# konstantineder/montecarlo-risk-engine

Hardware: AMD Instinct MI355X
Metric: path-steps/sec at 1M paths x 250 steps; PV/CVA rel-error vs CPU ref (higher is better)
Workload: dtype f64

## Files before the change

### montecarlo-risk-engine_amd/csrc/kf_common.h

```cpp
#pragma once
#include <cstddef>
#include "mcx_device.h"



enum { FA_EXP = 1, FA_AFFINE = 2 };
struct FAtom {
    int32_t reg, parts;
    double a, d, b, c0, c1;
};
struct FTerm { double w; FAtom atom; };
enum { FE_SAME_NUM = 2 };
struct FEvent {
    int32_t kind, flags;
    int32_t term_begin, term_end;
    int32_t coeff_off, row;
    int32_t ns, sidx;
    int32_t init_state, n_states;
    double strike, sign;
    double aux[4];
    FAtom num, x;
};
struct FMetricOp {
    int32_t ns, m;
// ... 385 lines not shown
        if (row >= 0) {
#pragma unroll
            for (int q = 0; q < PPL; ++q) if (live[q]) a.expo[(int64_t)row * a.ld_out + i[q]] = e[q];
        }
    }
    if (flags & FD_METRIC) {
        const double thr = FD(thr);
        double u[PPL];
#pragma unroll
        for (int q = 0; q < PPL; ++q) u[q] = dev_thr(e[q], thr);
        if (flags & FD_PROFILE) {
            const int rp = FD(rec_profile);
            double up[PPL], un[PPL];
#pragma unroll
            for (int q = 0; q < PPL; ++q) { up[q] = fmax(u[q], 0.0); un[q] = fmin(u[q], 0.0); }
            lean_record<PPL>(up, live, rp, a.n_rec, first_tile, lds);
            lean_record<PPL>(un, live, rp + 1, a.n_rec, first_tile, lds);
        }
        if (flags & FD_CVA) {
            const double sb = FD(s_b), sc0 = FD(s_c0), sc1 = FD(s_c1);
            const int sr = FD(s_reg);
            double sp[PPL], cs[PPL];
#pragma unroll
            for (int q = 0; q < PPL; ++q) sp[q] = sb * mcx_exp_tab(fma(sc1, reg[q][sr], sc0), etab, ec);
            cond_surv(cs);
#pragma unroll
            for (int q = 0; q < PPL; ++q) cva[q] = fma(fmax(u[q], 0.0), sp[q] * (1.0 - cs[q]), cva[q]);
        }
    }
}

#undef FD

int mcx_launch_kf_lean(const FusedArgs& a, const mcx_sim_desc& sd, int n_cu, bool inject, bool simulate, hipStream_t s);
```

### montecarlo-risk-engine_amd/csrc/kf_fused.hip

```cpp
#include "kf_common.h"

#include <algorithm>
#include <type_traits>
#include <cmath>
#include <cstdlib>

namespace {

template <int NSLOT, int SIG, int NNS, int NSTA, bool STORE>
__device__ __forceinline__ void kf_on_date(KArgs& a, int t, int64_t i, bool live, bool first_tile, double* __restrict__ lds,
                                           const unsigned char* __restrict__ chunk, const double (&reg)[2 * NSLOT],
                                           double (&cfs)[NNS], double (&cva)[NNS], int (&est)[NSTA])
{
    constexpr int NREG = 2 * NSLOT;
    const auto& k = a.k1;
    const int n_rec = a.n_rec;
    if (STORE && k.paths && live) sim_store_state<NSLOT, SIG>(k, t, i, reg);
    const ChunkHeader* hdp = (const ChunkHeader*)chunk;
    ChunkHeader hd;
    hd.n_ev = RFL(hdp->n_ev); hd.n_mop = RFL(hdp->n_mop); hd.n_terms = RFL(hdp->n_terms); hd.bytes = 0;
    const FEvent* __restrict__ evs = (const FEvent*)(chunk + sizeof(ChunkHeader));
    const FTerm* __restrict__ terms = (const FTerm*)(evs + hd.n_ev);
    const FMetricOp* __restrict__ mops = (const FMetricOp*)(terms + hd.n_terms);
    double e_ns[NNS];
// ... 281 lines not shown
void launch_kf(const FusedArgs& a, int grid, size_t lds, const KfRoute& r, bool simulate, hipStream_t s)
{
    const int npf = r.npf;
#define MCX_KF(INJ, NNS, NST, NPF) do { if (simulate) hipLaunchKernelGGL((kf_fused<NSLOT, NZ, INJ, SIG, NNS, NST, NPF, true>), dim3(grid), dim3(MCX_BLOCK), lds, s, a); \
        else if (!INJ) hipLaunchKernelGGL((kf_fused<NSLOT, NZ, false, SIG, NNS, NST, NPF, false>), dim3(grid), dim3(MCX_BLOCK), lds, s, a); } while (0)
#define MCX_KF_NPF(INJ, NNS, NST) do { if (npf == 1) MCX_KF(INJ, NNS, NST, 1); else if (npf == 2) MCX_KF(INJ, NNS, NST, 2); else MCX_KF(INJ, NNS, NST, 0); } while (0)
    if (r.inject) {
        if (r.nns == 1 && r.nst == 0) MCX_KF_NPF(true, 1, 0);
        else if (r.nns == 1) MCX_KF(true, 1, MCX_FUSED_MAX_STATEFUL, 0);
        else MCX_KF(true, MCX_FUSED_MAX_NS, MCX_FUSED_MAX_STATEFUL, 0);
    } else {
        if (r.nns == 1 && r.nst == 0) MCX_KF_NPF(false, 1, 0);
        else if (r.nns == 1) MCX_KF_NPF(false, 1, MCX_FUSED_MAX_STATEFUL);
        else MCX_KF(false, MCX_FUSED_MAX_NS, MCX_FUSED_MAX_STATEFUL, 0);
    }
#undef MCX_KF_NPF
#undef MCX_KF
}

}

struct mcx_fused {
    const mcx_sim* sim = nullptr;
    const mcx_book* book = nullptr;
    int n_rec = 0, n_ns = 0, n_dates = 0, n_expo_rows = 0, n_stateful = 0, want_pv = 0;
    unsigned char* d_prog = nullptr;
    FastDate* d_fast = nullptr;
    int32_t* d_date_off = nullptr;
    int32_t* d_date_row = nullptr;
    int chunk_cap = 0, npf = 0, max_chunk = 0;
    int lean = 0;
    FastDateCva* d_cva = nullptr;
    int cva_steps = 0;
    LeanTerm* d_lterms = nullptr;
    double* d_vcoef = nullptr;
    int32_t rec_pv[MCX_FUSED_MAX_NS] = {}, rec_cva[MCX_FUSED_MAX_NS] = {};
    double lgd[MCX_FUSED_MAX_NS] = {};
    int32_t init_state[MCX_FUSED_MAX_STATEFUL] = {};
    std::vector<int32_t> date_desc;
    double* d_partials = nullptr;
    size_t partial_bytes = 0;
    mcx_acc* d_out = nullptr;
    mutable hipEvent_t tev[2 * MCX_FUSED_TIMING_RING] = {};
    mutable int timing = 0, t_count = 0, t_launch = 0;
};

static void fused_timing_off(mcx_fused* f)
{
    if (f->timing) for (int q = 0; q < 2 * MCX_FUSED_TIMING_RING; ++q) hipEventDestroy(f->tev[q]);
    f->timing = 0; f->t_count = 0; f->t_launch = 0;
}

extern "C" int mcx_fused_set_timing(mcx_fused* f, int32_t enable)
{
    if (!f) return -1;
    fused_timing_off(f);
    if (enable) {
        for (int q = 0; q < 2 * MCX_FUSED_TIMING_RING; ++q)
            if (hipEventCreate(&f->tev[q]) != hipSuccess) { for (int r = 0; r < q; ++r) hipEventDestroy(f->tev[r]); return -100; }
        f->timing = enable > 0 ? enable : 1;
    }
    return 0;
}

extern "C" int mcx_fused_kernel_times(mcx_fused* f, float* h_ms, int32_t capacity, int32_t* n_out)
{
    if (!f || !h_ms || !n_out) return -1;
    *n_out = 0;
    if (!f->timing) return 0;
    const int n = f->t_count < capacity ? f->t_count : capacity;
    for (int q = 0; q < n; ++q) {
        if (hipEventSynchronize(f->tev[2 * q + 1]) != hipSuccess) return -100;
        if (hipEventElapsedTime(&h_ms[q], f->tev[2 * q], f->tev[2 * q + 1]) != hipSuccess) return -100;
    }
    *n_out = n;
    f->t_count = 0; f->t_launch = 0;
    return 0;
}

extern "C" void mcx_fused_destroy(mcx_fused* f)
{
    if (!f) return;
    fused_timing_off(f);
    hipFree(f->d_lterms); hipFree(f->d_vcoef); hipFree(f->d_cva); hipFree(f->d_prog); hipFree(f->d_fast); hipFree(f->d_date_off); hipFree(f->d_date_row); hipFree(f->d_partials); hipFree(f->d_out);
    delete f;
}

extern "C" int mcx_fused_num_records(const mcx_fused* f) { return f ? f->n_rec : -1; }

namespace {

struct FusedPlan {
    std::vector<unsigned char> prog;
    std::vector<FastDate> fast;
    std::vector<FastDateCva> cva_dates;
    std::vector<LeanTerm> lterms;
    std::vector<double> vcoef;
    std::vector<int32_t> date_off, date_row;
    int n_rec = 0, n_stateful = 0, npf = 0, chunk_cap = 0, max_chunk = 0, cva_steps = 0;
    bool lean = false, cva_only = false;
    int32_t rec_pv[MCX_FUSED_MAX_NS], rec_cva[MCX_FUSED_MAX_NS];
    double lgd[MCX_FUSED_MAX_NS];
    int32_t init_state[MCX_FUSED_MAX_STATEFUL] = {};
};

struct DateLists {
    std::vector<std::vector<FEvent>> events;
    std::vector<std::vector<int>> event_q;
    std::vector<std::vector<FTerm>> terms;
    std::vector<std::vector<FMetricOp>> mops;
    explicit DateLists(int T) : events(T), event_q(T), terms(T), mops(T) {}
};

struct Refusal {
    bool ok = true;
    std::string why;
    void operator()(const char* reason) { ok = false; why = reason; }
};

int check_arguments(mcx_handle* h, const mcx_sim_desc& sd, const mcx_book* book, const mcx_fused_desc* d)
{
    if (book->n_state != sd.n_state) MCX_FAIL(h, -2, "mcx_fused_create: book and sim disagree on the state dimension");
    if (d->n_netting_sets < 1 || d->n_netting_sets > MCX_FUSED_MAX_NS || d->n_netting_sets != book->n_netting_sets)
        MCX_FAIL(h, MCX_E_NOT_FUSABLE, "not fusable: %d netting sets (max %d)", book->n_netting_sets, MCX_FUSED_MAX_NS);
    if (d->n_expo_rows != book->n_expo_rows) MCX_FAIL(h, -2, "mcx_fused_create: n_expo_rows mismatch");
    for (int s = 0; s < sd.n_slots; ++s)
        if (sd.slots[s].kind == MCX_MODEL_S2F) MCX_FAIL(h, MCX_E_NOT_FUSABLE, "not fusable: the Schwartz two-factor spot is a derived state column");
    if ((int)book->h_event_t_idx.size() != book->n_events) MCX_FAIL(h, -2, "mcx_fused_create: internal (event dates missing)");
    return 0;
}

void state_registers(const mcx_sim_desc& sd, int (&col_reg)[MCX_MAX_STATE])
{
// ... 270 lines not shown
    p.date_off[T] = (int32_t)p.prog.size();
    p.prog.resize(p.prog.size() + 4096, 0);
    p.npf = p.max_chunk == 0 ? 0 : (p.max_chunk <= 1024 ? 1 : (p.max_chunk <= 2048 ? 2 : 0));
    p.chunk_cap = p.npf > 0 ? p.npf * 1024 : ((p.max_chunk + 255) & ~255);
}

bool straight_line_book(const mcx_sim_desc& sd, const mcx_fused_desc& d, const FusedPlan& p)
{
    bool lean = d.n_netting_sets == 1 && p.n_stateful <= 1;
    for (const FastDate& fd : p.fast) lean = lean && fd.valid != 0;
    for (int q = 0; q < sd.n_slots; ++q)
        if (sd.slots[q].kind == MCX_MODEL_CIRPP && !(sd.init_state[sd.slots[q].state_off] > 0.0)) lean = false;
    return lean;
}

bool is_cva_increment(const FastDate& fd) { return (fd.flags & (FD_MERGED | FD_EXERCISE | FD_STATE_EXPO)) == FD_MERGED; }

void build_cva_dates(const mcx_sim& sim, const mcx_book& book, FusedPlan& p)
{
    const int T = (int)p.fast.size();
    p.cva_dates.resize(T);
    p.cva_only = p.lean && mcx_sim_signature(sim.desc) == SIG_VAS_CIR_E && p.rec_pv[0] < 0 && p.rec_cva[0] >= 0 && book.n_basis == 3;
    for (int t = 0; t < T && p.cva_only; ++t) {
        const FastDate& fd = p.fast[t];
        FastDateCva& c = p.cva_dates[t];
        memset(&c, 0, sizeof(c));
        c.coeff_off0 = c.coeff_off1 = -1;
        if (is_cva_increment(fd)) {
            p.cva_only = fd.c_b != 0.0 && fd.s_reg == FDC_S_REG && fd.ni_reg == FDC_NI_REG && fd.c_reg == FDC_C_REG && fd.x_reg == FDC_X_REG;
            c.m_s1 = fd.m_s1; c.m_n1 = fd.m_n1; c.m_c0 = fd.m_c0; c.m_b = fd.m_b;
            c.c_c1 = fd.c_c1; c.c_c0 = fd.c_c0; c.c_a = fd.c_a; c.c_b = fd.c_b;
            c.x_d = fd.x_d; c.x_a = fd.x_a;
            if (fd.flags & FD_EXPO) { c.coeff_off0 = fd.coeff_off0; c.coeff_off1 = fd.coeff_off1; }
        } else if (fd.flags & (FD_METRIC | FD_EXERCISE | FD_STATE_EXPO)) {
            p.cva_only = false;
        }
    }
    int cva_steps = 0;
    for (size_t k = 0; k < sim.h_steps.size() && p.cva_only; ++k) {
        const int st = sim.h_steps[k].store_idx;
        if (st >= 0 && st < T && is_cva_increment(p.fast[st])) cva_steps = (int)k + 1;
    }
    p.cva_steps = cva_steps > 0 ? cva_steps : (int)sim.h_steps.size();
}

int upload(mcx_handle* h, const mcx_sim* sim, const mcx_book* book, const mcx_fused_desc& d, const FusedPlan& p, mcx_fused** out)
{
    mcx_fused* f = new mcx_fused();
    f->sim = sim; f->book = book; f->n_rec = p.n_rec; f->n_ns = d.n_netting_sets; f->n_dates = (int)p.fast.size(); f->n_expo_rows = d.n_expo_rows;
    f->n_stateful = p.n_stateful; f->want_pv = d.want_pv;
    f->npf = p.npf; f->chunk_cap = p.chunk_cap; f->max_chunk = p.max_chunk; f->lean = p.lean ? 1 : 0; f->cva_steps = p.cva_steps;
    for (int k = 0; k < MCX_FUSED_MAX_NS; ++k) { f->rec_pv[k] = p.rec_pv[k]; f->rec_cva[k] = p.rec_cva[k]; f->lgd[k] = p.lgd[k]; }
    for (int q = 0; q < MCX_FUSED_MAX_STATEFUL; ++q) f->init_state[q] = p.init_state[q];
    for (const FastDate& fd : p.fast) { f->date_desc.push_back(fd.valid); f->date_desc.push_back(fd.flags); }
    auto up = [&](auto** dst, const auto& src) -> hipError_t {
        const size_t bytes = sizeof(src[0]) * src.size();
        hipError_t e = hipMalloc((void**)dst, bytes ? bytes : 8);
        if (e != hipSuccess) return e;
        return bytes ? hipMemcpy(*dst, src.data(), bytes, hipMemcpyHostToDevice) : hipSuccess;
    };
    f->partial_bytes = sizeof(double) * 4 * (size_t)p.n_rec * 2048;
    hipError_t e = up(&f->d_prog, p.prog);
    if (e == hipSuccess) e = up(&f->d_fast, p.fast);
    if (e == hipSuccess && p.cva_only) e = up(&f->d_cva, p.cva_dates);
    if (e == hipSuccess) e = up(&f->d_lterms, p.lterms);
    if (e == hipSuccess) e = up(&f->d_vcoef, p.vcoef);
    if (e == hipSuccess) e = up(&f->d_date_off, p.date_off);
    if (e == hipSuccess) e = up(&f->d_date_row, p.date_row);
    if (e == hipSuccess) e = hipMalloc(&f->d_partials, f->partial_bytes);
    if (e == hipSuccess) e = hipMalloc(&f->d_out, sizeof(mcx_acc) * (size_t)p.n_rec);
    if (e != hipSuccess) {
        mcx_fused_destroy(f);
        MCX_FAIL(h, -100 - (int)e, "mcx_fused_create: %s", hipGetErrorString(e));
    }
    *out = f;
    return 0;
}

}

extern "C" int mcx_fused_create(mcx_handle* h, const mcx_sim* sim, const mcx_book* book, const mcx_fused_desc* d, mcx_fused** out)
{
    if (!h || !sim || !book || !d || !out) return -1;
    MCX_REFUSE_WIDE(h, sim, "mcx_fused_create");
// ... 54 lines not shown
    if (!h || !f || (h_out == nullptr) == (d_out == nullptr)) return -1;
    if (n_paths <= 0) {
        if (h_out) memset(h_out, 0, sizeof(mcx_acc) * (size_t)f->n_rec);
        else MCX_HIP(h, hipMemsetAsync(d_out, 0, sizeof(mcx_acc) * (size_t)f->n_rec, (hipStream_t)stream));
        return 0;
    }
    if ((d_paths || d_inject_z) && ld < n_paths) MCX_FAIL(h, -2, "mcx_fused_run: ld < n_paths");
    if ((d_cfs || d_expo) && ld_out < n_paths) MCX_FAIL(h, -2, "mcx_fused_run: ld_out < n_paths");
    if ((size_t)f->n_rec * sizeof(mcx_acc) > h->pinned_bytes) MCX_FAIL(h, -2, "mcx_fused_run: too many records");
    const mcx_sim_desc& sd = f->sim->desc;
    if (sd.n_uniform && d_inject_z && !d_inject_u) MCX_FAIL(h, -3, "mcx_fused_run: inject_u required with inject_z under QE");
    if (!simulate && (!d_paths || ld < n_paths)) MCX_FAIL(h, -2, "mcx_fused_eval_paths: a paths tensor with ld >= n_paths is required");
    FusedArgs a;
    memset(&a, 0, sizeof(a));
    mcx_fill_k1_args(f->sim, seed, path_offset, n_paths, ld > 0 ? ld : n_paths, d_paths, d_inject_z, d_inject_u, &a.k1);
    a.cva_dates = (simulate && !d_inject_z && !d_paths && !d_cfs && !d_expo) ? f->d_cva : nullptr;
    if (a.cva_dates) a.k1.n_steps = f->cva_steps;
    a.prog = f->d_prog; a.fast = f->d_fast; a.lterms = f->d_lterms; a.vcoef = f->d_vcoef; a.date_off = f->d_date_off; a.chunk_cap = f->chunk_cap;
    a.date_row = f->d_date_row; a.coeffs = f->book->d_coeffs; a.cfs = d_cfs; a.expo = d_expo; a.partials = f->d_partials;
    a.ld_out = ld_out; a.n_dates = f->n_dates; a.n_basis = f->book->n_basis; a.n_ns = f->n_ns; a.n_rec = f->n_rec;
    a.n_expo_rows = f->n_expo_rows; a.n_stateful = f->n_stateful;
    for (int k = 0; k < MCX_FUSED_MAX_NS; ++k) { a.rec_pv[k] = f->rec_pv[k]; a.rec_cva[k] = f->rec_cva[k]; a.lgd[k] = f->lgd[k]; }
    for (int k = 0; k < MCX_FUSED_MAX_STATEFUL; ++k) a.init_state[k] = f->init_state[k];
    hipStream_t s = (hipStream_t)stream;
    const bool inj = d_inject_z != nullptr;
    int grid;
    const bool timed = f->timing && (f->t_launch++ % f->timing) == 0 && f->t_count < MCX_FUSED_TIMING_RING;
    if (timed) MCX_HIP(h, hipEventRecord(f->tev[2 * f->t_count], s));
    const bool direct = !d_out && sizeof(mcx_acc) * (size_t)f->n_rec <= h->pinned_bytes && h->d_pinned_alias;
    mcx_acc* dst = d_out ? d_out : (direct ? (mcx_acc*)h->d_pinned_alias : f->d_out);
    const KfRoute route = kf_route(f, inj, simulate);
    if (route.kernel == MCX_ROUTE_NONE) MCX_FAIL(h, -2, "mcx_fused_run: no kernel evaluates a paths tensor with injected draws");
    if (route.kernel == MCX_ROUTE_LEAN) {
        grid = mcx_launch_kf_lean(a, sd, h->n_cu, inj, simulate, s);
        if (grid < 0) MCX_FAIL(h, MCX_E_NOT_FUSABLE, "not fusable: (slots=%d, z=%d) has no fused instantiation", sd.n_slots, sd.n_z);
    } else {
        const int64_t tiles = (n_paths + MCX_BLOCK - 1) / MCX_BLOCK;
        grid = (int)std::min<int64_t>(tiles, 2048);
        if (tiles > 2048) { int per = (int)((tiles + 2047) / 2048); grid = (int)((tiles + per - 1) / per); }
        const size_t lds = sizeof(double) * (size_t)((9 * f->n_rec + 1) & ~1) + (size_t)4 * f->chunk_cap;
        const bool launched = mcx_dispatch_signature<4>(sd, [&](auto nslot, auto nz, auto sig) {
            launch_kf<decltype(nslot)::value, decltype(nz)::value, decltype(sig)::value>(a, grid, lds, route, simulate, s);
        });
        if (!launched) MCX_FAIL(h, MCX_E_NOT_FUSABLE, "not fusable: (slots=%d, z=%d) has no fused instantiation", sd.n_slots, sd.n_z);
    }
    MCX_HIP(h, hipGetLastError());
    if (timed) { MCX_HIP(h, hipEventRecord(f->tev[2 * f->t_count + 1], s)); ++f->t_count; }
    hipLaunchKernelGGL(kf_merge, dim3(f->n_rec), dim3(MCX_BLOCK), 0, s, f->d_partials, f->n_rec, grid, dst);
    MCX_HIP(h, hipGetLastError());
    if (d_out) return 0;
    if (!direct) MCX_HIP(h, hipMemcpyAsync(h->h_pinned, f->d_out, sizeof(mcx_acc) * (size_t)f->n_rec, hipMemcpyDeviceToHost, s));
    MCX_HIP(h, hipStreamSynchronize(s));
    memcpy(h_out, h->h_pinned, sizeof(mcx_acc) * (size_t)f->n_rec);
    return 0;
}

extern "C" int mcx_fused_is_straight_line(const mcx_fused* f)
{
    return (f && f->lean) ? 1 : 0;
}

extern "C" int mcx_fused_describe(const mcx_fused* f, int32_t inject, int32_t simulate, int32_t* out, int32_t cap)
{
    if (!f || cap < 0 || (cap > 0 && !out)) return -1;
    const int need = MCX_FDESC_HEADER + 2 * f->n_dates;
    if (cap < need) return need;
    const KfRoute r = kf_route(f, inject != 0, simulate != 0);
// ... 36 lines not shown
```

### montecarlo-risk-engine_amd/csrc/kf_lean.hip

```cpp
#include <cstdlib>
#include <map>
#include <utility>

#include "kf_common.h"

namespace {

template <int NSLOT, int PPL>
__device__ __forceinline__ void lean_date_cva(const FastDateCvaLds* __restrict__ rp, const double (&reg)[PPL][2 * NSLOT], double (&cva)[PPL],
                                              const double* __restrict__ etab)
{
    const mcx_expq_coef ec = mcx_expq_load(mcx_region_zero());
    const FastDateCvaLds r = *rp;
    double xe[2 * PPL], ev[2 * PPL];
#pragma unroll
    for (int q = 0; q < PPL; ++q) {
        xe[2 * q] = fma(r.m_s1, reg[q][FDC_S_REG], fma(r.m_n1, reg[q][FDC_NI_REG], r.m_c0));
        xe[2 * q + 1] = fma(r.c_c1, reg[q][FDC_C_REG], r.c_c0);
    }
    mcx_exp_tab_n<2 * PPL>(xe, ev, etab, ec);
#pragma unroll
    for (int q = 0; q < PPL; ++q) {
        const double x = fma(r.x_d, reg[q][FDC_X_REG], r.x_a);
        double p = 0.0;
        p += fma(fma(r.row0[2], x, r.row0[1]), x, r.row0[0]);
        p += fma(fma(r.row1[2], x, r.row1[1]), x, r.row1[0]);
        const double w = r.m_b * ev[2 * q];
        const double cs = fma(r.c_b, ev[2 * q + 1], r.c_a);
        cva[q] = fma(fmax(p, 0.0), w * (1.0 - cs), cva[q]);
    }
}

template <int PPL>
__device__ __forceinline__ void philox4x32_10_cva(const uint32_t (&path_lo)[PPL], uint32_t path_hi, uint32_t step, uint32_t draw, uint64_t seed,
                                                  uint32_t (&o0)[PPL], uint32_t (&o1)[PPL], uint32_t (&o2)[PPL], uint32_t (&o3)[PPL])
{
    constexpr uint32_t M0 = 0xD2511F53u, M1 = 0xCD9E8D57u, W0 = 0x9E3779B9u, W1 = 0xBB67AE85u;
    uint32_t k0 = (uint32_t)seed, k1 = (uint32_t)(seed >> 32);
    uint32_t c0[PPL], c1[PPL], c2[PPL], c3[PPL];
    const uint64_t s1 = (uint64_t)M1 * step;
    const uint32_t hk = path_hi ^ k0;
    const uint32_t a0 = (uint32_t)(s1 >> 32) ^ hk, a1 = (uint32_t)s1;
    const uint32_t dk = draw ^ k1;
#pragma unroll
    for (int q = 0; q < PPL; ++q) {
        const uint64_t p0 = (uint64_t)M0 * path_lo[q];
        c2[q] = (uint32_t)(p0 >> 32) ^ dk;
        c3[q] = (uint32_t)p0;
    }
    k0 += W0; k1 += W1;
    const uint64_t s0 = (uint64_t)M0 * a0;
#pragma unroll
    for (int q = 0; q < PPL; ++q) {
        const uint64_t p1 = (uint64_t)M1 * c2[q];
        c0[q] = ((uint32_t)(p1 >> 32) ^ k0) ^ a1;
        c2[q] = (c3[q] ^ k1) ^ (uint32_t)(s0 >> 32);
        c1[q] = (uint32_t)p1;
    }
    k0 += W0; k1 += W1;
    const uint32_t x3 = (uint32_t)s0 ^ k1;
#pragma unroll
    for (int q = 0; q < PPL; ++q) {
        const uint64_t p0 = (uint64_t)M0 * c0[q];
        const uint64_t p1 = (uint64_t)M1 * c2[q];
        c0[q] = __builtin_amdgcn_bitop3_b32((uint32_t)(p1 >> 32), c1[q], k0, 0x96);
        c2[q] = (uint32_t)(p0 >> 32) ^ x3;
        c1[q] = (uint32_t)p1; c3[q] = (uint32_t)p0;
    }
    k0 += W0; k1 += W1;
#pragma unroll
    for (int r = 3; r < 10; ++r) {
#pragma unroll
        for (int q = 0; q < PPL; ++q) {
            const uint64_t p0 = (uint64_t)M0 * c0[q];
            const uint64_t p1 = (uint64_t)M1 * c2[q];
            const uint32_t n0 = __builtin_amdgcn_bitop3_b32((uint32_t)(p1 >> 32), c1[q], k0, 0x96);
            const uint32_t n2 = __builtin_amdgcn_bitop3_b32((uint32_t)(p0 >> 32), c3[q], k1, 0x96);
            c1[q] = (uint32_t)p1; c3[q] = (uint32_t)p0; c0[q] = n0; c2[q] = n2;
        }
        k0 += W0; k1 += W1;
    }
#pragma unroll
    for (int q = 0; q < PPL; ++q) { o0[q] = c0[q]; o1[q] = c1[q]; o2[q] = c2[q]; o3[q] = c3[q]; }
}

struct CvaDrawConst {
    double off52;
    double trig_scale;
};
__device__ __forceinline__ CvaDrawConst cva_draw_const_make()
{
    CvaDrawConst c;
    c.off52 = mcx_opaque_v(0x1.0p52 - 0.5); c.trig_scale = mcx_opaque_v(6.28318530717958647692 * 0x1.0p-53);
    return c;
}

template <int PPL, int BMB>
__device__ __forceinline__ bool cva_draw_pairs(uint64_t seed, const uint32_t (&path_lo)[PPL], uint32_t path_hi, uint32_t step, uint32_t draw,
                                               double (&z0)[PPL], double (&z1)[PPL], const double* __restrict__ tab,
                                               const mcx_bm_coef& C, const mcx_bm_vconst& vc, const CvaDrawConst& dc)
{
    static_assert(BMB >= 1 && BMB <= 20, "the funnel shift of the high word is by 11 + BMB < 32 bits");
    constexpr int N = 1 << BMB, LOG_TERMS = mcx_bm_shape<BMB>::LOG_TERMS;
    uint32_t w0[PPL], w1[PPL], w2[PPL], w3[PPL];
    philox4x32_10_cva<PPL>(path_lo, path_hi, step, draw, seed, w0, w1, w2, w3);
    double m[PPL], ed[PPL], ps[PPL], pc[PPL];
    int e[PPL];
    mcx_d2 tc[PPL], sc[PPL];
#pragma unroll
    for (int q = 0; q < PPL; ++q) {
        const double ua = u53(w0[q], w1[q], &vc);
        m[q] = __builtin_amdgcn_frexp_mant(ua);
        e[q] = __builtin_amdgcn_frexp_exp(ua);
        const int jl = (__double2hiint(m[q]) >> (20 - BMB)) & (N - 1);
        tc[q] = ((const mcx_d2*)tab)[jl];
        sc[q] = ((const mcx_d2*)(tab + 2 * N))[(int)(w3[q] >> (32 - BMB))];
    }
    __builtin_amdgcn_sched_barrier(0);
#pragma unroll
    for (int q = 0; q < PPL; ++q) {
        const uint32_t lo = __builtin_amdgcn_alignbit(w3[q], w2[q], 11);
        const uint32_t hi = __builtin_amdgcn_alignbit(0x43300000u >> (21 - BMB), w3[q] << BMB, 11 + BMB);
        const double v = __hiloint2double((int)hi, (int)lo) - dc.off52;
        const double d = fma(v, dc.trig_scale, vc.trig_off);
        const double d2 = d * d;
        double qs, qc;
        if constexpr (mcx_bm_shape<BMB>::TRIG_TERMS == 3) {
            qs = fma(fma(vc.sin_head, d2, C.c[7]), d2, C.c[6]);
            qc = fma(fma(vc.cos_head, d2, C.c[10]), d2, C.c[9]);
        } else {
            qs = fma(vc.sin_head, d2, C.c[6]);
            qc = fma(vc.cos_head, d2, C.c[9]);
        }
        ps[q] = fma(d * d2, qs, d);
        pc[q] = fma(d2, qc, 1.0);
        ed[q] = (double)e[q];
    }
    __builtin_amdgcn_sched_barrier(0);
    uint32_t top = 0;
#pragma unroll
    for (int q = 0; q < PPL; ++q) {
        const double s = fma(m[q], tc[q].x, 2.0);
        double p = vc.log_head;
#pragma unroll
        for (int k = LOG_TERMS - 2; k >= 0; --k) p = fma(p, s, C.c[k]);
        const double r2 = fma(ed[q], -2.0 * 6.93147180559945309417e-01, tc[q].y) + fma(s * s, p, s);
        const double r = mcx_sqrt_gp(r2);
        const double sn = fma(sc[q].x, pc[q], sc[q].y * ps[q]);
        const double cs = fma(-sc[q].x, ps[q], sc[q].y * pc[q]);
        z0[q] = r * cs;
        z1[q] = r * sn;
        top = w1[q] > top ? w1[q] : top;
    }
    return top == 0xffffffffu;
}

#define MCX_LEAN_WAVES 4
template <int NSLOT, int NZ, bool INJECT, int SIG, int PPL, bool SIMULATE, int DK = 0>
__global__ __launch_bounds__(MCX_BLOCK, MCX_LEAN_WAVES) void kf_lean(const FusedArgs)
{
    static_assert(DK == 0 || (SIG == SIG_VAS_CIR_E && SIMULATE && !INJECT), "the cva-date kernel simulates the Vasicek + CIR++ signature");
    constexpr int NREG = 2 * NSLOT;
    constexpr int TILE = MCX_BLOCK * PPL;
    extern __shared__ double lds[];
    KArgs& a0 = kargs_region(0);
    const int n_rec = a0.n_rec;
    const int64_t n = a0.k1.n;
    for (int q = threadIdx.x; q < 9 * n_rec; q += MCX_BLOCK) lds[q] = 0.0;
    FastDateCvaLds* const dlds = (FastDateCvaLds*)(lds + ((9 * n_rec + 1) & ~1));
    if constexpr (DK != 0) {
        const FastDateCva* __restrict__ dc = a0.cva_dates;
        const double* __restrict__ cf = a0.coeffs;
        const int n_dates = a0.n_dates;
        for (int q = threadIdx.x; q < 16 * n_dates; q += MCX_BLOCK) {
            const int t = q >> 4, e = q & 15;
            double v;
            if (e < FDC_HEAD) {
                v = ((const double*)(dc + t))[e];
            } else {
                const int off = e < FDC_HEAD + 3 ? dc[t].coeff_off0 : dc[t].coeff_off1;
                v = off >= 0 ? cf[off + (e - FDC_HEAD) % 3] : 0.0;
            }
            ((double*)dlds)[q] = v;
        }
    }
    constexpr int BMB = SIG == SIG_VAS_CIR_E ? 10 : 7;
    constexpr int BM = (INJECT || !SIMULATE) ? 0 : MCX_BM_LDS_DOUBLES_B(BMB);
    __shared__ double tab_lds[BM + MCX_EXP_LDS_DOUBLES];
    const double* tab = nullptr;
    const double* etab = tab_lds + BM;
    mcx_exp_tab_load(tab_lds + BM);
    if (BM) { mcx_bm_load<BMB>(tab_lds); tab = tab_lds; }
    __syncthreads();
    const int64_t tiles = (n + TILE - 1) / TILE;
    double n_block = 0.0;

    for (int64_t tile = blockIdx.x; tile < tiles; tile += gridDim.x) {
        const bool first_tile = tile == (int64_t)blockIdx.x;
        int64_t i[PPL];
        bool live[PPL];
        uint64_t path[PPL];
        double reg[PPL][NREG];
        double cfs[PPL], cva[PPL];
        int est[PPL];
        int n_init, n_steps;
        {
            KArgs& a = kargs_region(mcx_region_zero());
            const auto& k = a.k1;
#pragma unroll
            for (int q = 0; q < PPL; ++q) {
                const int64_t i_raw = tile * TILE + q * MCX_BLOCK + threadIdx.x;
                live[q] = i_raw < n;
                i[q] = live[q] ? i_raw : n - 1;
                path[q] = k.path_offset + (uint64_t)i[q];
                sim_init_state<NSLOT, SIG>(k, reg[q]);
                cfs[q] = 0.0; cva[q] = 0.0;
                est[q] = a.init_state[0];
            }
            const int64_t rest = n - tile * TILE;
            n_block += (double)(rest < TILE ? rest : TILE);
            n_init = k.n_initial_store; n_steps = k.n_steps;
        }
        if (SIMULATE) {
        int step = 0, t_init = 0;
#pragma unroll 1
        while (true) {
            const bool init = t_init < n_init;
            if (!init && step >= n_steps) break;
            int st = init ? t_init : -1;
            t_init += init ? 1 : 0;
            {
                const int zr0 = mcx_region_zero();
                const auto& k = kargs_region(zr0).k1;
                const uint64_t seed = k.seed;
                const mcx_bm_coef bc = mcx_bm_coef_load(zr0);
                const mcx_bm_vconst vc = mcx_bm_vconst_make<BMB>(bc);
                uint32_t path_hi = 0;
                CvaDrawConst dc = {};
                if constexpr (DK == 1) { path_hi = ((const MCX_KONST uint32_t*)&k.path_offset)[1]; dc = cva_draw_const_make(); }
#pragma unroll 1
                while (st < 0 && step < n_steps) {
                    if constexpr (SIG == SIG_GENERIC) {
#pragma unroll
                        for (int q = 0; q < PPL; ++q) sim_substep<NSLOT, NZ, INJECT, SIG, BMB, true>(k, step, path[q], i[q], reg[q], tab, seed, bc, &vc);
                        st = ldk(&k.steps[step].store_idx);
                    } else {
                        double zz[PPL][NZ], uu[PPL];
                        bool rare = false;
                        const StepData<NSLOT, NZ> sdat = sim_step_load<NSLOT, NZ, SIG>(k, step);
                        __builtin_amdgcn_sched_barrier(0);
                        if constexpr (INJECT) {
#pragma unroll
                            for (int q = 0; q < PPL; ++q) sim_draw<NZ, true, SIG, BMB>(k, step, path[q], i[q], zz[q], uu[q], tab, seed, bc, &vc);
                        } else if constexpr (DK == 1) {
                            static_assert(NZ == 2, "one Philox block per path and sub-step");
                            uint32_t plo[PPL];
                            double za[PPL], zb[PPL];
#pragma unroll
                            for (int q = 0; q < PPL; ++q) plo[q] = (uint32_t)path[q];
                            rare = cva_draw_pairs<PPL, BMB>(seed, plo, path_hi, (uint32_t)step, 0u, za, zb, tab, bc, vc, dc);
#pragma unroll
                            for (int q = 0; q < PPL; ++q) { zz[q][0] = za[q]; zz[q][1] = zb[q]; uu[q] = 0.0; }
                        } else {
                            uint32_t st_q[PPL];
#pragma unroll
                            for (int q = 0; q < PPL; ++q) st_q[q] = (uint32_t)step;
                            rare = sim_draw_n<PPL, NZ, SIG, BMB>(k, st_q, path, zz, uu, tab, seed, bc, vc);
                        }
                        if (!INJECT && __builtin_expect(__any(rare), 0)) {
                            if constexpr (DK == 1) {
#pragma unroll
                                for (int q = 0; q < PPL; ++q)
                                    sim_draw<NZ, false, SIG, BMB, true>(k, step, ((uint64_t)path_hi << 32) | (uint32_t)path[q], i[q], zz[q], uu[q], tab, seed, bc, &vc);
                            } else {
#pragma unroll
                                for (int q = 0; q < PPL; ++q) sim_draw<NZ, false, SIG, BMB, true>(k, step, path[q], i[q], zz[q], uu[q], tab, seed, bc, &vc);
                            }
                        }
#pragma unroll
                        for (int q = 0; q < PPL; ++q) st = sim_apply_loaded<NSLOT, NZ, SIG, true>(k, sdat, reg[q], zz[q], uu[q]);
                    }
                    ++step;
                }
            }
            if (st >= 0) {
                if constexpr (DK != 0) lean_date_cva<NSLOT, PPL>(dlds + st, reg, cva, etab);
                else lean_date<NSLOT, SIG, PPL, true>(st, i, live, first_tile, lds, reg, cfs, cva, est, etab);
            }
        }
        } else {
            auto load_row = [&](int t, double (&dst)[PPL][NREG]) {
                const auto& k = kargs_region(0).k1;
                const int D = k.n_state;
#pragma unroll
                for (int q = 0; q < PPL; ++q)
#pragma unroll
                    for (int sl = 0; sl < NSLOT; ++sl) {
                        const bool bs = sig_kind(SIG, sl) >= 0 ? sig_is_bs(SIG, sl) : (k.slots[sl].kind == MCX_MODEL_BS);
                        const int c = k.slots[sl].state_off;
                        dst[q][2 * sl] = k.paths[((int64_t)t * D + c) * k.ld + i[q]];
                        dst[q][2 * sl + 1] = bs ? 0.0 : k.paths[((int64_t)t * D + c + 1) * k.ld + i[q]];
                    }
            };
            const int n_dates = kargs_region(0).n_dates;
            double bufb[PPL][NREG];
            load_row(0, reg);
            load_row(n_dates > 1 ? 1 : 0, bufb);
#pragma unroll 1
            for (int t = 0; t < n_dates; t += 2) {
                lean_date<NSLOT, SIG, PPL, false>(t, i, live, first_tile, lds, reg, cfs, cva, est, etab);
                if (t + 2 < n_dates) load_row(t + 2, reg);
                if (t + 1 < n_dates) {
                    lean_date<NSLOT, SIG, PPL, false>(t + 1, i, live, first_tile, lds, bufb, cfs, cva, est, etab);
                    if (t + 3 < n_dates) load_row(t + 3, bufb);
                }
            }
        }
        {
            KArgs& a = kargs_region(mcx_region_zero());
#pragma unroll
            for (int q = 0; q < PPL; ++q) if (a.cfs && live[q]) a.cfs[i[q]] = cfs[q];
            if (a.rec_pv[0] >= 0) lean_record<PPL>(cfs, live, a.rec_pv[0], n_rec, first_tile, lds);
            if (a.rec_cva[0] >= 0) {
                const double lgd = a.lgd[0];
                double cc[PPL];
#pragma unroll
                for (int q = 0; q < PPL; ++q) cc[q] = cva[q] * lgd;
                lean_record<PPL>(cc, live, a.rec_cva[0], n_rec, first_tile, lds);
            }
        }
    }
    __syncthreads();
    for (int r = threadIdx.x; r < n_rec; r += MCX_BLOCK) {
        double s1 = 0.0, s2 = 0.0;
        for (int w = 0; w < 4; ++w) { s1 += lds[n_rec + (w * n_rec + r) * 2]; s2 += lds[n_rec + (w * n_rec + r) * 2 + 1]; }
        double* dst = a0.partials + ((int64_t)blockIdx.x * n_rec + r) * 4;
        dst[0] = n_block; dst[1] = lds[r]; dst[2] = s1; dst[3] = s2;
    }
}

template <int NSLOT, int NZ, int SIG, int PPL>
int launch_lean_shape(const FusedArgs& a, int full_steps, int n_cu, bool inject, bool simulate, hipStream_t s)
{
    const int64_t tiles = (a.k1.n + MCX_BLOCK * PPL - 1) / (MCX_BLOCK * PPL);
    const size_t lds = sizeof(double) * (size_t)((9 * a.n_rec + 1) & ~1);
    const size_t lds_cva = lds + sizeof(FastDateCvaLds) * (size_t)a.n_dates;
    auto residency = [&](auto kernel, size_t bytes) {
        thread_local std::map<std::pair<const void*, size_t>, int> cache;
        const auto key = std::make_pair((const void*)kernel, bytes);
        auto it = cache.find(key);
        if (it == cache.end()) {
            int per_cu = 0;
            if (hipOccupancyMaxActiveBlocksPerMultiprocessor(&per_cu, kernel, MCX_BLOCK, bytes) != hipSuccess || per_cu < 1) per_cu = 1;
            it = cache.emplace(key, per_cu < MCX_LEAN_WAVES ? per_cu : MCX_LEAN_WAVES).first;
        }
        return (int64_t)it->second * n_cu;
    };
    auto sized = [&](int64_t resident) {
        if (tiles <= resident) return (int)tiles;
        const int64_t per = (tiles + resident - 1) / resident;
        return (int)((tiles + per - 1) / per);
    };
    int grid;
    if (!simulate) {
        auto kern = kf_lean<NSLOT, NZ, false, SIG, PPL, false>;
        grid = sized(residency(kern, lds));
        hipLaunchKernelGGL(kern, dim3(grid), dim3(MCX_BLOCK), lds, s, a);
    } else if (inject) {
        auto kern = kf_lean<NSLOT, NZ, true, SIG, PPL, true>;
        grid = sized(residency(kern, lds));
        hipLaunchKernelGGL(kern, dim3(grid), dim3(MCX_BLOCK), lds, s, a);
    } else {
        auto kern = kf_lean<NSLOT, NZ, false, SIG, PPL, true>;
        const int64_t resident = residency(kern, lds);
        if constexpr (SIG == SIG_VAS_CIR_E) {
            auto kern_cva = kf_lean<NSLOT, NZ, false, SIG, 2, true, 1>;
            auto kern_cva_thin = kf_lean<NSLOT, NZ, false, SIG, PPL, true, 2>;
            const bool one_high_word = ((a.k1.path_offset + (uint64_t)(a.k1.n - 1)) >> 32) == (a.k1.path_offset >> 32);
            if (a.cva_dates && one_high_word) {
                grid = sized(resident);
                if (PPL == 2 && grid >= resident) {
                    if (residency(kern_cva, lds_cva) >= resident) {
                        hipLaunchKernelGGL(kern_cva, dim3(grid), dim3(MCX_BLOCK), lds_cva, s, a);
                        return grid;
                    }
                } else if (residency(kern_cva_thin, lds_cva) >= resident) {
                    hipLaunchKernelGGL(kern_cva_thin, dim3(grid), dim3(MCX_BLOCK), lds_cva, s, a);
                    return grid;
                }
            }
        }
        grid = sized(resident);
        FusedArgs g = a;
        g.k1.n_steps = full_steps;
        hipLaunchKernelGGL(kern, dim3(grid), dim3(MCX_BLOCK), lds, s, g);
    }
    return grid;
}

template <int NSLOT, int NZ, int SIG>
void launch_lean(const FusedArgs& a, int full_steps, int n_cu, bool inject, bool simulate, hipStream_t s, int* grid_out)
{
    constexpr int PPL = (SIG == SIG_GENERIC && NSLOT >= 2) ? 1 : 2;
#ifdef MCX_LEAN_AB
    if (simulate && !inject) {
        const char* sh = getenv("MCX_LEAN_SHAPE");
        const int code = sh ? atoi(sh) : 0;
        if (code == 11) { *grid_out = launch_lean_shape<NSLOT, NZ, SIG, 1>(a, full_steps, n_cu, inject, simulate, s); return; }
        if (code == 21) { *grid_out = launch_lean_shape<NSLOT, NZ, SIG, 2>(a, full_steps, n_cu, inject, simulate, s); return; }
    }
#endif
    const int64_t full_tiles = (a.k1.n + MCX_BLOCK * PPL - 1) / (MCX_BLOCK * PPL);
    if (PPL == 2 && simulate && !inject && full_tiles < (int64_t)2 * n_cu) {
        *grid_out = launch_lean_shape<NSLOT, NZ, SIG, 1>(a, full_steps, n_cu, inject, simulate, s);
        return;
    }
    *grid_out = launch_lean_shape<NSLOT, NZ, SIG, PPL>(a, full_steps, n_cu, inject, simulate, s);
}

}

int mcx_launch_kf_lean(const FusedArgs& a, const mcx_sim_desc& sd, int n_cu, bool inject, bool simulate, hipStream_t s)
{
    int grid = -1;
#ifdef MCX_LEAN_ONE_SIG
    if (mcx_sim_signature(sd) == SIG_VAS_CIR_E) launch_lean<2, 2, SIG_VAS_CIR_E>(a, sd.n_steps, n_cu, inject, simulate, s, &grid);
#else
    mcx_dispatch_signature<4>(sd, [&](auto nslot, auto nz, auto sig) {
        launch_lean<decltype(nslot)::value, decltype(nz)::value, decltype(sig)::value>(a, sd.n_steps, n_cu, inject, simulate, s, &grid);
    });
#endif
    return grid;
}
```

Baseline: 311.4 billion.

## Specialise CVA kernel for one-row dates and hoist per-lane Philox round

Adds a ROWS template parameter so the CVA-date kernel skips the second regression polynomial when no date uses a second coefficient row, selected on the host from the date plan. The path-dependent part of the first Philox round is computed once per lane before the step loop instead of on every step. The rare-path fallback now reuses the Philox words already generated rather than regenerating them. The table index is computed directly as a byte offset. Together these trim per-step integer multiplies and per-date FMAs, at the cost of extra registers held across the loop and one more kernel instantiation.

```diff
diff --git a/montecarlo-risk-engine_amd/csrc/kf_common.h b/montecarlo-risk-engine_amd/csrc/kf_common.h
--- a/montecarlo-risk-engine_amd/csrc/kf_common.h
+++ b/montecarlo-risk-engine_amd/csrc/kf_common.h
@@ -441,4 +441,4 @@
 
 #undef FD
 
-int mcx_launch_kf_lean(const FusedArgs& a, const mcx_sim_desc& sd, int n_cu, bool inject, bool simulate, hipStream_t s);
+int mcx_launch_kf_lean(const FusedArgs& a, const mcx_sim_desc& sd, int cva_rows, int n_cu, bool inject, bool simulate, hipStream_t s);
diff --git a/montecarlo-risk-engine_amd/csrc/kf_fused.hip b/montecarlo-risk-engine_amd/csrc/kf_fused.hip
--- a/montecarlo-risk-engine_amd/csrc/kf_fused.hip
+++ b/montecarlo-risk-engine_amd/csrc/kf_fused.hip
@@ -337,6 +337,7 @@
     int lean = 0;
     FastDateCva* d_cva = nullptr;
     int cva_steps = 0;
+    int cva_rows = 2;
     LeanTerm* d_lterms = nullptr;
     double* d_vcoef = nullptr;
     int32_t rec_pv[MCX_FUSED_MAX_NS] = {}, rec_cva[MCX_FUSED_MAX_NS] = {};
@@ -403,7 +404,7 @@
     std::vector<double> vcoef;
     std::vector<int32_t> date_off, date_row;
     int n_rec = 0, n_stateful = 0, npf = 0, chunk_cap = 0, max_chunk = 0, cva_steps = 0;
-    bool lean = false, cva_only = false;
+    bool lean = false, cva_only = false, cva_two_rows = false;
     int32_t rec_pv[MCX_FUSED_MAX_NS], rec_cva[MCX_FUSED_MAX_NS];
     double lgd[MCX_FUSED_MAX_NS];
     int32_t init_state[MCX_FUSED_MAX_STATEFUL] = {};
@@ -740,6 +741,7 @@
             c.c_c1 = fd.c_c1; c.c_c0 = fd.c_c0; c.c_a = fd.c_a; c.c_b = fd.c_b;
             c.x_d = fd.x_d; c.x_a = fd.x_a;
             if (fd.flags & FD_EXPO) { c.coeff_off0 = fd.coeff_off0; c.coeff_off1 = fd.coeff_off1; }
+            if (c.coeff_off1 >= 0) p.cva_two_rows = true;
         } else if (fd.flags & (FD_METRIC | FD_EXERCISE | FD_STATE_EXPO)) {
             p.cva_only = false;
         }
@@ -757,7 +759,7 @@
     mcx_fused* f = new mcx_fused();
     f->sim = sim; f->book = book; f->n_rec = p.n_rec; f->n_ns = d.n_netting_sets; f->n_dates = (int)p.fast.size(); f->n_expo_rows = d.n_expo_rows;
     f->n_stateful = p.n_stateful; f->want_pv = d.want_pv;
-    f->npf = p.npf; f->chunk_cap = p.chunk_cap; f->max_chunk = p.max_chunk; f->lean = p.lean ? 1 : 0; f->cva_steps = p.cva_steps;
+    f->npf = p.npf; f->chunk_cap = p.chunk_cap; f->max_chunk = p.max_chunk; f->lean = p.lean ? 1 : 0; f->cva_steps = p.cva_steps; f->cva_rows = p.cva_two_rows ? 2 : 1;
     for (int k = 0; k < MCX_FUSED_MAX_NS; ++k) { f->rec_pv[k] = p.rec_pv[k]; f->rec_cva[k] = p.rec_cva[k]; f->lgd[k] = p.lgd[k]; }
     for (int q = 0; q < MCX_FUSED_MAX_STATEFUL; ++q) f->init_state[q] = p.init_state[q];
     for (const FastDate& fd : p.fast) { f->date_desc.push_back(fd.valid); f->date_desc.push_back(fd.flags); }
@@ -878,7 +880,7 @@
     const KfRoute route = kf_route(f, inj, simulate);
     if (route.kernel == MCX_ROUTE_NONE) MCX_FAIL(h, -2, "mcx_fused_run: no kernel evaluates a paths tensor with injected draws");
     if (route.kernel == MCX_ROUTE_LEAN) {
-        grid = mcx_launch_kf_lean(a, sd, h->n_cu, inj, simulate, s);
+        grid = mcx_launch_kf_lean(a, sd, f->cva_rows, h->n_cu, inj, simulate, s);
         if (grid < 0) MCX_FAIL(h, MCX_E_NOT_FUSABLE, "not fusable: (slots=%d, z=%d) has no fused instantiation", sd.n_slots, sd.n_z);
     } else {
         const int64_t tiles = (n_paths + MCX_BLOCK - 1) / MCX_BLOCK;
diff --git a/montecarlo-risk-engine_amd/csrc/kf_lean.hip b/montecarlo-risk-engine_amd/csrc/kf_lean.hip
--- a/montecarlo-risk-engine_amd/csrc/kf_lean.hip
+++ b/montecarlo-risk-engine_amd/csrc/kf_lean.hip
@@ -6,7 +6,7 @@
 
 namespace {
 
-template <int NSLOT, int PPL>
+template <int NSLOT, int PPL, int ROWS>
 __device__ __forceinline__ void lean_date_cva(const FastDateCvaLds* __restrict__ rp, const double (&reg)[PPL][2 * NSLOT], double (&cva)[PPL],
                                               const double* __restrict__ etab)
 {
@@ -22,9 +22,14 @@
 #pragma unroll
     for (int q = 0; q < PPL; ++q) {
         const double x = fma(r.x_d, reg[q][FDC_X_REG], r.x_a);
-        double p = 0.0;
-        p += fma(fma(r.row0[2], x, r.row0[1]), x, r.row0[0]);
-        p += fma(fma(r.row1[2], x, r.row1[1]), x, r.row1[0]);
+        double p;
+        if constexpr (ROWS == 1) {
+            p = fma(fma(r.row0[2], x, r.row0[1]), x, r.row0[0]);
+        } else {
+            p = 0.0;
+            p += fma(fma(r.row0[2], x, r.row0[1]), x, r.row0[0]);
+            p += fma(fma(r.row1[2], x, r.row1[1]), x, r.row1[0]);
+        }
         const double w = r.m_b * ev[2 * q];
         const double cs = fma(r.c_b, ev[2 * q + 1], r.c_a);
         cva[q] = fma(fmax(p, 0.0), w * (1.0 - cs), cva[q]);
@@ -32,7 +37,27 @@
 }
 
 template <int PPL>
-__device__ __forceinline__ void philox4x32_10_cva(const uint32_t (&path_lo)[PPL], uint32_t path_hi, uint32_t step, uint32_t draw, uint64_t seed,
+struct CvaLaneWords { uint32_t h0[PPL], c1[PPL], c3[PPL]; };
+template <int PPL>
+__device__ __forceinline__ CvaLaneWords<PPL> philox_cva_lane(const uint32_t (&path_lo)[PPL], uint32_t draw, uint64_t seed)
+{
+    constexpr uint32_t M0 = 0xD2511F53u, M1 = 0xCD9E8D57u, W0 = 0x9E3779B9u, W1 = 0xBB67AE85u;
+    const uint32_t k0 = (uint32_t)seed, k1 = (uint32_t)(seed >> 32);
+    const uint32_t dk = draw ^ k1;
+    CvaLaneWords<PPL> L;
+#pragma unroll
+    for (int q = 0; q < PPL; ++q) {
+        const uint64_t p0 = (uint64_t)M0 * path_lo[q];
+        const uint64_t p1 = (uint64_t)M1 * ((uint32_t)(p0 >> 32) ^ dk);
+        L.h0[q] = (uint32_t)(p1 >> 32) ^ (k0 + W0);
+        L.c1[q] = (uint32_t)p1;
+        L.c3[q] = (uint32_t)p0 ^ (k1 + W1);
+    }
+    return L;
+}
+
+template <int PPL>
+__device__ __forceinline__ void philox4x32_10_cva(const CvaLaneWords<PPL>& L, uint32_t path_hi, uint32_t step, uint64_t seed,
                                                   uint32_t (&o0)[PPL], uint32_t (&o1)[PPL], uint32_t (&o2)[PPL], uint32_t (&o3)[PPL])
 {
     constexpr uint32_t M0 = 0xD2511F53u, M1 = 0xCD9E8D57u, W0 = 0x9E3779B9u, W1 = 0xBB67AE85u;
@@ -41,21 +66,13 @@
     const uint64_t s1 = (uint64_t)M1 * step;
     const uint32_t hk = path_hi ^ k0;
     const uint32_t a0 = (uint32_t)(s1 >> 32) ^ hk, a1 = (uint32_t)s1;
-    const uint32_t dk = draw ^ k1;
-#pragma unroll
-    for (int q = 0; q < PPL; ++q) {
-        const uint64_t p0 = (uint64_t)M0 * path_lo[q];
-        c2[q] = (uint32_t)(p0 >> 32) ^ dk;
-        c3[q] = (uint32_t)p0;
-    }
     k0 += W0; k1 += W1;
     const uint64_t s0 = (uint64_t)M0 * a0;
 #pragma unroll
     for (int q = 0; q < PPL; ++q) {
-        const uint64_t p1 = (uint64_t)M1 * c2[q];
-        c0[q] = ((uint32_t)(p1 >> 32) ^ k0) ^ a1;
-        c2[q] = (c3[q] ^ k1) ^ (uint32_t)(s0 >> 32);
-        c1[q] = (uint32_t)p1;
+        c0[q] = L.h0[q] ^ a1;
+        c2[q] = L.c3[q] ^ (uint32_t)(s0 >> 32);
+        c1[q] = L.c1[q];
     }
     k0 += W0; k1 += W1;
     const uint32_t x3 = (uint32_t)s0 ^ k1;
@@ -96,14 +113,14 @@
 }
 
 template <int PPL, int BMB>
-__device__ __forceinline__ bool cva_draw_pairs(uint64_t seed, const uint32_t (&path_lo)[PPL], uint32_t path_hi, uint32_t step, uint32_t draw,
+__device__ __forceinline__ bool cva_draw_pairs(uint64_t seed, const CvaLaneWords<PPL>& lane, uint32_t path_hi, uint32_t step,
                                                double (&z0)[PPL], double (&z1)[PPL], const double* __restrict__ tab,
-                                               const mcx_bm_coef& C, const mcx_bm_vconst& vc, const CvaDrawConst& dc)
+                                               const mcx_bm_coef& C, const mcx_bm_vconst& vc, const CvaDrawConst& dc,
+                                               uint32_t (&w0)[PPL], uint32_t (&w1)[PPL], uint32_t (&w2)[PPL], uint32_t (&w3)[PPL])
 {
     static_assert(BMB >= 1 && BMB <= 20, "the funnel shift of the high word is by 11 + BMB < 32 bits");
     constexpr int N = 1 << BMB, LOG_TERMS = mcx_bm_shape<BMB>::LOG_TERMS;
-    uint32_t w0[PPL], w1[PPL], w2[PPL], w3[PPL];
-    philox4x32_10_cva<PPL>(path_lo, path_hi, step, draw, seed, w0, w1, w2, w3);
+    philox4x32_10_cva<PPL>(lane, path_hi, step, seed, w0, w1, w2, w3);
     double m[PPL], ed[PPL], ps[PPL], pc[PPL];
     int e[PPL];
     mcx_d2 tc[PPL], sc[PPL];
@@ -112,8 +129,8 @@
         const double ua = u53(w0[q], w1[q], &vc);
         m[q] = __builtin_amdgcn_frexp_mant(ua);
         e[q] = __builtin_amdgcn_frexp_exp(ua);
-        const int jl = (__double2hiint(m[q]) >> (20 - BMB)) & (N - 1);
-        tc[q] = ((const mcx_d2*)tab)[jl];
+        const uint32_t jb = ((uint32_t)__double2hiint(m[q]) >> (16 - BMB)) & ((N - 1) << 4);
+        tc[q] = *(const mcx_d2*)((const char*)tab + jb);
         sc[q] = ((const mcx_d2*)(tab + 2 * N))[(int)(w3[q] >> (32 - BMB))];
     }
     __builtin_amdgcn_sched_barrier(0);
@@ -156,10 +173,11 @@
 }
 
 #define MCX_LEAN_WAVES 4
-template <int NSLOT, int NZ, bool INJECT, int SIG, int PPL, bool SIMULATE, int DK = 0>
+template <int NSLOT, int NZ, bool INJECT, int SIG, int PPL, bool SIMULATE, int DK = 0, int ROWS = 2>
 __global__ __launch_bounds__(MCX_BLOCK, MCX_LEAN_WAVES) void kf_lean(const FusedArgs)
 {
     static_assert(DK == 0 || (SIG == SIG_VAS_CIR_E && SIMULATE && !INJECT), "the cva-date kernel simulates the Vasicek + CIR++ signature");
+    static_assert(ROWS == 2 || (ROWS == 1 && DK == 1), "only the full-grid cva-date kernel has a one-row date program");
     constexpr int NREG = 2 * NSLOT;
     constexpr int TILE = MCX_BLOCK * PPL;
     extern __shared__ double lds[];
@@ -203,6 +221,7 @@
         double reg[PPL][NREG];
         double cfs[PPL], cva[PPL];
         int est[PPL];
+        CvaLaneWords<PPL> lane_words;
         int n_init, n_steps;
         {
             KArgs& a = kargs_region(mcx_region_zero());
@@ -220,6 +239,13 @@
             const int64_t rest = n - tile * TILE;
             n_block += (double)(rest < TILE ? rest : TILE);
             n_init = k.n_initial_store; n_steps = k.n_steps;
+            if constexpr (DK == 1) {
+                static_assert(NZ == 2, "one Philox block per path and sub-step: draw index 0");
+                uint32_t plo[PPL];
+#pragma unroll
+                for (int q = 0; q < PPL; ++q) plo[q] = (uint32_t)path[q];
+                lane_words = philox_cva_lane<PPL>(plo, 0u, k.seed);
+            }
         }
         if (SIMULATE) {
         int step = 0, t_init = 0;
@@ -246,6 +272,7 @@
                         st = ldk(&k.steps[step].store_idx);
                     } else {
                         double zz[PPL][NZ], uu[PPL];
+                        uint32_t w0[PPL], w1[PPL], w2[PPL], w3[PPL];
                         bool rare = false;
                         const StepData<NSLOT, NZ> sdat = sim_step_load<NSLOT, NZ, SIG>(k, step);
                         __builtin_amdgcn_sched_barrier(0);
@@ -253,12 +280,8 @@
 #pragma unroll
                             for (int q = 0; q < PPL; ++q) sim_draw<NZ, true, SIG, BMB>(k, step, path[q], i[q], zz[q], uu[q], tab, seed, bc, &vc);
                         } else if constexpr (DK == 1) {
-                            static_assert(NZ == 2, "one Philox block per path and sub-step");
-                            uint32_t plo[PPL];
                             double za[PPL], zb[PPL];
-#pragma unroll
-                            for (int q = 0; q < PPL; ++q) plo[q] = (uint32_t)path[q];
-                            rare = cva_draw_pairs<PPL, BMB>(seed, plo, path_hi, (uint32_t)step, 0u, za, zb, tab, bc, vc, dc);
+                            rare = cva_draw_pairs<PPL, BMB>(seed, lane_words, path_hi, (uint32_t)step, za, zb, tab, bc, vc, dc, w0, w1, w2, w3);
 #pragma unroll
                             for (int q = 0; q < PPL; ++q) { zz[q][0] = za[q]; zz[q][1] = zb[q]; uu[q] = 0.0; }
                         } else {
@@ -270,8 +293,10 @@
                         if (!INJECT && __builtin_expect(__any(rare), 0)) {
                             if constexpr (DK == 1) {
 #pragma unroll
-                                for (int q = 0; q < PPL; ++q)
-                                    sim_draw<NZ, false, SIG, BMB, true>(k, step, ((uint64_t)path_hi << 32) | (uint32_t)path[q], i[q], zz[q], uu[q], tab, seed, bc, &vc);
+                                for (int q = 0; q < PPL; ++q) {
+                                    double ua;
+                                    pair_from_words<true, BMB, true>(w0[q], w1[q], w2[q], w3[q], ua, zz[q][0], zz[q][1], tab, bc, &vc);
+                                }
                             } else {
 #pragma unroll
                                 for (int q = 0; q < PPL; ++q) sim_draw<NZ, false, SIG, BMB, true>(k, step, path[q], i[q], zz[q], uu[q], tab, seed, bc, &vc);
@@ -284,7 +309,7 @@
                 }
             }
             if (st >= 0) {
-                if constexpr (DK != 0) lean_date_cva<NSLOT, PPL>(dlds + st, reg, cva, etab);
+                if constexpr (DK != 0) lean_date_cva<NSLOT, PPL, ROWS>(dlds + st, reg, cva, etab);
                 else lean_date<NSLOT, SIG, PPL, true>(st, i, live, first_tile, lds, reg, cfs, cva, est, etab);
             }
         }
@@ -340,7 +365,7 @@
 }
 
 template <int NSLOT, int NZ, int SIG, int PPL>
-int launch_lean_shape(const FusedArgs& a, int full_steps, int n_cu, bool inject, bool simulate, hipStream_t s)
+int launch_lean_shape(const FusedArgs& a, int full_steps, int cva_rows, int n_cu, bool inject, bool simulate, hipStream_t s)
 {
     const int64_t tiles = (a.k1.n + MCX_BLOCK * PPL - 1) / (MCX_BLOCK * PPL);
     const size_t lds = sizeof(double) * (size_t)((9 * a.n_rec + 1) & ~1);
@@ -374,7 +399,8 @@
         auto kern = kf_lean<NSLOT, NZ, false, SIG, PPL, true>;
         const int64_t resident = residency(kern, lds);
         if constexpr (SIG == SIG_VAS_CIR_E) {
-            auto kern_cva = kf_lean<NSLOT, NZ, false, SIG, 2, true, 1>;
+            auto kern_cva = cva_rows == 1 ? kf_lean<NSLOT, NZ, false, SIG, 2, true, 1, 1>
+                                          : kf_lean<NSLOT, NZ, false, SIG, 2, true, 1, 2>;
             auto kern_cva_thin = kf_lean<NSLOT, NZ, false, SIG, PPL, true, 2>;
             const bool one_high_word = ((a.k1.path_offset + (uint64_t)(a.k1.n - 1)) >> 32) == (a.k1.path_offset >> 32);
             if (a.cva_dates && one_high_word) {
@@ -399,35 +425,35 @@
 }
 
 template <int NSLOT, int NZ, int SIG>
-void launch_lean(const FusedArgs& a, int full_steps, int n_cu, bool inject, bool simulate, hipStream_t s, int* grid_out)
+void launch_lean(const FusedArgs& a, int full_steps, int cva_rows, int n_cu, bool inject, bool simulate, hipStream_t s, int* grid_out)
 {
     constexpr int PPL = (SIG == SIG_GENERIC && NSLOT >= 2) ? 1 : 2;
 #ifdef MCX_LEAN_AB
     if (simulate && !inject) {
         const char* sh = getenv("MCX_LEAN_SHAPE");
         const int code = sh ? atoi(sh) : 0;
-        if (code == 11) { *grid_out = launch_lean_shape<NSLOT, NZ, SIG, 1>(a, full_steps, n_cu, inject, simulate, s); return; }
-        if (code == 21) { *grid_out = launch_lean_shape<NSLOT, NZ, SIG, 2>(a, full_steps, n_cu, inject, simulate, s); return; }
+        if (code == 11) { *grid_out = launch_lean_shape<NSLOT, NZ, SIG, 1>(a, full_steps, cva_rows, n_cu, inject, simulate, s); return; }
+        if (code == 21) { *grid_out = launch_lean_shape<NSLOT, NZ, SIG, 2>(a, full_steps, cva_rows, n_cu, inject, simulate, s); return; }
     }
 #endif
     const int64_t full_tiles = (a.k1.n + MCX_BLOCK * PPL - 1) / (MCX_BLOCK * PPL);
     if (PPL == 2 && simulate && !inject && full_tiles < (int64_t)2 * n_cu) {
-        *grid_out = launch_lean_shape<NSLOT, NZ, SIG, 1>(a, full_steps, n_cu, inject, simulate, s);
+        *grid_out = launch_lean_shape<NSLOT, NZ, SIG, 1>(a, full_steps, cva_rows, n_cu, inject, simulate, s);
         return;
     }
-    *grid_out = launch_lean_shape<NSLOT, NZ, SIG, PPL>(a, full_steps, n_cu, inject, simulate, s);
-}
-
-}
-
-int mcx_launch_kf_lean(const FusedArgs& a, const mcx_sim_desc& sd, int n_cu, bool inject, bool simulate, hipStream_t s)
+    *grid_out = launch_lean_shape<NSLOT, NZ, SIG, PPL>(a, full_steps, cva_rows, n_cu, inject, simulate, s);
+}
+
+}
+
+int mcx_launch_kf_lean(const FusedArgs& a, const mcx_sim_desc& sd, int cva_rows, int n_cu, bool inject, bool simulate, hipStream_t s)
 {
     int grid = -1;
 #ifdef MCX_LEAN_ONE_SIG
-    if (mcx_sim_signature(sd) == SIG_VAS_CIR_E) launch_lean<2, 2, SIG_VAS_CIR_E>(a, sd.n_steps, n_cu, inject, simulate, s, &grid);
+    if (mcx_sim_signature(sd) == SIG_VAS_CIR_E) launch_lean<2, 2, SIG_VAS_CIR_E>(a, sd.n_steps, cva_rows, n_cu, inject, simulate, s, &grid);
 #else
     mcx_dispatch_signature<4>(sd, [&](auto nslot, auto nz, auto sig) {
-        launch_lean<decltype(nslot)::value, decltype(nz)::value, decltype(sig)::value>(a, sd.n_steps, n_cu, inject, simulate, s, &grid);
+        launch_lean<decltype(nslot)::value, decltype(nz)::value, decltype(sig)::value>(a, sd.n_steps, cva_rows, n_cu, inject, simulate, s, &grid);
     });
 #endif
     return grid;
```

New measurement: 318.6 billion, median of 6. +2.3%, better.
